# Newiz430/CellSegmentation

Measured on AMD Instinct MI355X. Metric: tiles/sec fwd+bwd (ResNet-50 MIL, 299x299), higher is better.
Workload: dtype bf16; 1 GPU; ResNet-50 tile classifier (train_tile.py --scratch semantics: fwd + CE + full bwd + Adam), bag=64 tiles of 299x299x3 per GPU, freeze_bn=True; tiles_per_gpu=64, parallelism=dp1

## Files before the change

### cellsegmentation_amd/_lib.py

```python
import ctypes
import os
from ctypes import POINTER, Structure, c_char_p, c_double, c_float, c_int, c_int32, c_int64, c_longlong, c_size_t, c_void_p

_HERE = os.path.dirname(os.path.abspath(__file__))
FLAVOUR = os.environ.get("CELLSEG_LIB_FLAVOUR", "")
if FLAVOUR not in ("", "ab"):
    raise RuntimeError(f"CELLSEG_LIB_FLAVOUR={FLAVOUR!r}: expected unset or 'ab'")
LIB_PATH = os.path.join(_HERE, f"libcellseg_hip_{FLAVOUR}.so" if FLAVOUR else "libcellseg_hip.so")

CS_F32, CS_BF16 = 0, 1
CS_ACT_NONE, CS_ACT_RELU, CS_ACT_SILU, CS_ACT_SIGMOID = 0, 1, 2, 3
CS_BN_BWD_OWN_RELU, CS_BN_BWD_FROZEN = 0x100, 0x200


class CsConvGeom(Structure):
    _fields_ = [(n, c_int32) for n in ("N", "H", "W", "C", "K", "R", "S", "stride", "pad", "P", "Q", "groups")]


class CsStageDesc(Structure):
    _fields_ = ([(n, c_void_p) for n in ("w", "gamma", "beta", "mean", "var", "conv_bias", "w_khwc", "w_chwk", "scale", "shift", "rstd")]
                + [("eps", c_float)] + [(n, c_int32) for n in ("K", "Cin", "R", "S", "Cp", "Kp", "block0", "fwd_packed", "bwd_packed")])


class CellsegLibraryMissing(RuntimeError):
# ... 34 lines not shown
    "cs_conv2d_wgrad_batched_splits": (c_int, [POINTER(CsConvGeom), c_int, c_int]),
    "cs_conv2d_wgrad2_supported": (c_int, [POINTER(CsConvGeom), c_int]),
    "cs_conv2d_wgrad_batched": (c_int, [POINTER(CsConvGeom), c_int, _P, _P, _P, c_int, c_int, _P]),
    "cs_wgrad_finalize_batched": (c_int, [_P, _P, c_int, c_int, c_int, c_int, c_int, c_int, c_int, c_int, c_int, c_int, _P]),
    "cs_conv2d_dgrad_partial_rows": (c_int, [POINTER(CsConvGeom)]),
    "cs_fold_partial_rows": (c_int, [_P, c_int, c_int, _P, _P]),
    "cs_wgrad_finalize_grouped": (c_int, [_P, c_int, _P, _P, _P, _P, _P, c_int, c_int, c_int, c_int, _P, _P, _P, _P, _P]),
    "cs_colsum": (c_int, [_P, c_int, c_longlong, c_int, _P, _P]),
    "cs_colsum_partial_rows": (c_int, [c_longlong]),
    "cs_colsum_partial": (c_int, [_P, c_int, c_longlong, c_int, _P, _P]),
    "cs_positive_bits": (c_int, [_P, c_int, c_longlong, c_int, _P, _P]),
    "cs_adam_chunk_elems": (c_int, []),
    "cs_adam_max_tensors": (c_int, []),
    "cs_adam_step": (c_int, [_P, _P, c_int, c_int, _P, c_int, c_double, c_double, c_double, c_double, c_double, c_double, _P]),
    "cs_adam_step_dev": (c_int, [_P, _P, c_int, c_int, _P, c_int, _P, _P, _P, c_double, c_double, c_double, c_double, c_double, _P]),
    "cs_sgd_step": (c_int, [_P, _P, c_int, c_int, _P, c_int, c_double, c_double, c_double, c_double, c_int, c_int, _P]),
    "cs_sgd_step_dev": (c_int, [_P, _P, c_int, c_int, _P, c_int, _P, c_double, c_double, c_int, c_int, _P]),
    "cs_sample_sum_workspace": (c_size_t, [c_int, c_int, c_int]),
    "cs_sample_sum": (c_int, [_P, _P, c_int, c_float, _P, _P, c_int, c_int, c_int, _P]),
    "cs_maxpool3x3s2_fwd": (c_int, [_P, c_int, _P, _P, c_int, c_int, c_int, c_int, c_int, c_int, _P]),
    "cs_maxpool3x3s2_bwd": (c_int, [_P, _P, _P, c_int, _P, c_int, c_int, c_int, c_int, c_int, c_int, _P]),
    "cs_gap_avgmax_fwd": (c_int, [_P, c_int, _P, _P, c_int, c_int, c_int, c_int, _P]),
    "cs_gap_avgmax_bwd": (c_int, [_P, _P, _P, c_int, _P, c_int, c_int, c_int, c_int, c_int, _P]),
    "cs_linear_fwd": (c_int, [_P, _P, _P, _P, _P, c_int, c_int, c_int, c_int, _P]),
    "cs_linear_bwd_workspace": (c_size_t, [c_int, c_int, c_int]),
    "cs_linear_bwd": (c_int, [_P, _P, _P, _P, c_int, _P, _P, _P, c_int, c_int, c_int, c_int, _P, _P]),
    "cs_loss_words": (c_int, []),
    "cs_softmax_ce": (c_int, [_P, _P, c_float, _P, _P, c_int, c_int, _P]),
    "cs_softmax_prob1": (c_int, [_P, _P, c_int, c_int, _P]),
    "cs_softmax_argmax": (c_int, [_P, _P, c_int, c_int, _P]),
    "cs_mse": (c_int, [_P, _P, c_int, c_int, _P, _P, c_int, _P]),
    "cs_bn_accum_words": (c_size_t, [c_int]),
    "cs_bn_accum_read": (c_int, [_P, c_int, _P, _P]),
    "cs_bn_stats": (c_int, [_P, c_int, c_longlong, c_int, _P, _P, _P]),
    "cs_bn_partial_workspace": (c_size_t, [c_longlong, c_int]),
    "cs_bn_finalize": (c_int, [_P, c_longlong, c_float, c_float, _P, _P, _P, _P, c_int, _P]),
    "cs_bn_apply": (c_int, [_P, c_int, _P, _P, _P, _P, _P, c_int, _P, c_longlong, c_int, _P]),
    "cs_bn_apply_stats": (c_int, [_P, c_int, _P, c_float, c_float, _P, _P, _P, _P, _P, c_int, _P, _P, _P, c_longlong, c_int, _P]),
    "cs_bn_bwd_reduce": (c_int, [_P, _P, c_int, _P, _P, _P, _P, c_int, c_longlong, c_int, _P, _P, _P]),
    "cs_bn_bwd_apply": (c_int, [_P, _P, c_int, _P, _P, _P, _P, c_int, _P, c_longlong, c_int, _P, _P, _P, _P]),
    "cs_dwconv_fwd": (c_int, [POINTER(CsConvGeom), c_int, _P, _P, _P, _P, c_int, _P, _P]),
    "cs_dwconv_fwd_stats_workspace": (c_size_t, [POINTER(CsConvGeom)]),
    "cs_dwconv_fwd_stats": (c_int, [POINTER(CsConvGeom), c_int, _P, _P, _P, _P, POINTER(c_int), _P]),
    "cs_bn_partial_fold": (c_int, [_P, c_int, c_int, _P, _P]),
    "cs_dwconv_dgrad": (c_int, [POINTER(CsConvGeom), c_int, _P, _P, _P, _P]),
    "cs_dwconv_wgrad": (c_int, [POINTER(CsConvGeom), c_int, _P, _P, _P, _P, _P]),
# ... 143 lines not shown
```

### cellsegmentation_amd/csrc/pool.hip

```cpp
#include "cs_common.h"

namespace {

template <typename T>
__global__ __launch_bounds__(256) void maxpool_fwd_kernel(const T* __restrict__ x, T* __restrict__ y,
                                                          uint8_t* __restrict__ amax, int N, int H, int W, int C, int P,
                                                          int Q) {
    const int CG = C / 8;
    const long long total = (long long)N * P * Q * CG;
    for (long long idx = (long long)blockIdx.x * blockDim.x + threadIdx.x; idx < total;
         idx += (long long)gridDim.x * blockDim.x) {
        const int cg = (int)(idx % CG);
        long long t = idx / CG;
        const int q = (int)(t % Q); t /= Q;
        const int p = (int)(t % P);
        const long long n = t / P;
        float best[8];
        int bi[8];
#pragma unroll
        for (int e = 0; e < 8; ++e) { best[e] = -INFINITY; bi[e] = 0; }
        bool first = true;
#pragma unroll
        for (int kh = 0; kh < 3; ++kh) {
            const int iy = p * 2 - 1 + kh;
// ... 2 lines not shown
            for (int kw = 0; kw < 3; ++kw) {
                const int ix = q * 2 - 1 + kw;
                if (ix < 0 || ix >= W) continue;
                float v[8];
                load8<T>(x + ((n * H + iy) * (long long)W + ix) * C + cg * 8, v);
#pragma unroll
                for (int e = 0; e < 8; ++e) {
                    if (first || v[e] > best[e] || v[e] != v[e]) { best[e] = v[e]; bi[e] = kh * 3 + kw; }
                }
                first = false;
            }
        }
        const long long o = ((n * P + p) * (long long)Q + q) * C + cg * 8;
        store8<T>(y + o, best);
        if (amax) {
            uint2 pk;
            pk.x = (uint32_t)bi[0] | ((uint32_t)bi[1] << 8) | ((uint32_t)bi[2] << 16) | ((uint32_t)bi[3] << 24);
            pk.y = (uint32_t)bi[4] | ((uint32_t)bi[5] << 8) | ((uint32_t)bi[6] << 16) | ((uint32_t)bi[7] << 24);
            *reinterpret_cast<uint2*>(amax + o) = pk;
        }
    }
}

template <typename T>
__global__ __launch_bounds__(256) void maxpool_bwd_block_kernel(const T* __restrict__ dy, const uint8_t* __restrict__ amax,
                                                                const T* __restrict__ y, T* __restrict__ dx, int N, int H, int W,
                                                                int C, int P, int Q) {
    const int CG = C / 8;
    const int Ha = (H + 1) / 2, Wb = (W + 1) / 2;
    const long long total = (long long)N * Ha * Wb * CG;
    for (long long idx = (long long)blockIdx.x * blockDim.x + threadIdx.x; idx < total;
         idx += (long long)gridDim.x * blockDim.x) {
        const int cg = (int)(idx % CG);
        long long t = idx / CG;
        const int b = (int)(t % Wb); t /= Wb;
        const int a = (int)(t % Ha);
        const long long n = t / Ha;
        float acc[2][2][8];
#pragma unroll
        for (int i = 0; i < 2; ++i)
#pragma unroll
            for (int j = 0; j < 2; ++j)
#pragma unroll
                for (int e = 0; e < 8; ++e) acc[i][j][e] = 0.f;
#pragma unroll
        for (int wp = 0; wp < 2; ++wp) {
            const int p = a + wp;
            if (p >= P) continue;
#pragma unroll
            for (int wq = 0; wq < 2; ++wq) {
                const int q = b + wq;
// ... 6 lines not shown
                    float yy[8];
                    load8<T>(y + o, yy);
#pragma unroll
                    for (int e = 0; e < 8; ++e) g[e] = yy[e] > 0.f ? g[e] : 0.f;
                }
#pragma unroll
                for (int i = 0; i < 2; ++i) {
                    const int kh = i + 1 - 2 * wp;
                    if (kh < 0 || kh > 2) continue;
#pragma unroll
                    for (int j = 0; j < 2; ++j) {
                        const int kw = j + 1 - 2 * wq;
                        if (kw < 0 || kw > 2) continue;
                        const uint32_t want = (uint32_t)(kh * 3 + kw);
#pragma unroll
                        for (int e = 0; e < 8; ++e) {
                            const uint32_t am = ((e < 4 ? pk.x : pk.y) >> (8 * (e & 3))) & 0xffu;
                            if (am == want) acc[i][j][e] += g[e];
                        }
                    }
                }
            }
        }
#pragma unroll
        for (int i = 0; i < 2; ++i) {
            const int iy = 2 * a + i;
            if (iy >= H) continue;
#pragma unroll
            for (int j = 0; j < 2; ++j) {
                const int ix = 2 * b + j;
                if (ix < W) store8<T>(dx + ((n * H + iy) * (long long)W + ix) * C + cg * 8, acc[i][j]);
            }
        }
    }
}

template <typename T>
__global__ __launch_bounds__(256) void gap_fwd_kernel(const T* __restrict__ x, float* __restrict__ feat,
                                                      int32_t* __restrict__ amax, int HW, int C, int with_max) {
    const int CG = C / 8;
    const int n = blockIdx.y;
    const int cg = blockIdx.x * 64 + (threadIdx.x & 63);
    const int part = threadIdx.x >> 6;
    __shared__ float s_sum[4][64][8];
    __shared__ float s_max[4][64][8];
    __shared__ int s_idx[4][64][8];
    float sum[8], mx[8];
    int mi[8];
#pragma unroll
    for (int e = 0; e < 8; ++e) { sum[e] = 0.f; mx[e] = -INFINITY; mi[e] = 0x7fffffff; }
    if (cg < CG) {
        const T* base = x + (long long)n * HW * C + cg * 8;
        int p = part;
        for (; p + 12 < HW; p += 16) {
            float v[4][8];
#pragma unroll
            for (int u = 0; u < 4; ++u) load8<T>(base + (long long)(p + 4 * u) * C, v[u]);
// ... 19 lines not shown
    for (int e = 0; e < 8; ++e) {
        s_sum[part][threadIdx.x & 63][e] = sum[e];
        s_max[part][threadIdx.x & 63][e] = mx[e];
        s_idx[part][threadIdx.x & 63][e] = mi[e];
    }
    __syncthreads();
    if (part == 0 && cg < CG) {
        const int l = threadIdx.x & 63;
#pragma unroll
        for (int e = 0; e < 8; ++e) {
            float s = 0.f, m = -INFINITY;
            int bi = 0x7fffffff;
            for (int q = 0; q < 4; ++q) {
                s += s_sum[q][l][e];
                const float mq = s_max[q][l][e];
                const int iq = s_idx[q][l][e];
                if (iq == 0x7fffffff) continue;
                const bool nq = mq != mq, nm = m != m;
                if (bi == 0x7fffffff || (nq ? (!nm || iq > bi) : (!nm && (mq > m || (mq == m && iq < bi))))) { m = mq; bi = iq; }
            }
            feat[(long long)n * C + cg * 8 + e] = s / (float)HW + (with_max ? m : 0.f);
            if (amax) amax[(long long)n * C + cg * 8 + e] = bi;
        }
    }
}

template <typename T>
__global__ __launch_bounds__(256) void gap_bwd_kernel(const float* __restrict__ dfeat, const int32_t* __restrict__ amax,
                                                      const T* __restrict__ x, T* __restrict__ dx, int N, int HW, int C,
                                                      int relu_mask, int with_max) {
    const int CG = C / 8;
    const long long total = (long long)N * HW * CG;
    const float inv = 1.f / (float)HW;
    for (long long idx = (long long)blockIdx.x * blockDim.x + threadIdx.x; idx < total;
         idx += (long long)gridDim.x * blockDim.x) {
        const int cg = (int)(idx % CG);
        const long long t = idx / CG;
        const int p = (int)(t % HW);
        const long long n = t / HW;
        float v[8], g8[8];
        load8p(dfeat + n * C + cg * 8, 0.f, g8);
        int am[8];
        if (with_max) {
            const int4 a0 = *reinterpret_cast<const int4*>(amax + n * C + cg * 8);
            const int4 a1 = *reinterpret_cast<const int4*>(amax + n * C + cg * 8 + 4);
            am[0] = a0.x; am[1] = a0.y; am[2] = a0.z; am[3] = a0.w; am[4] = a1.x; am[5] = a1.y; am[6] = a1.z; am[7] = a1.w;
        }
#pragma unroll
        for (int e = 0; e < 8; ++e) v[e] = g8[e] * inv + ((with_max && am[e] == p) ? g8[e] : 0.f);
        const long long o = (n * HW + p) * C + cg * 8;
        if (relu_mask) {
            float xx[8];
            load8<T>(x + o, xx);
#pragma unroll
            for (int e = 0; e < 8; ++e) v[e] = xx[e] > 0.f ? v[e] : 0.f;
        }
        store8<T>(dx + o, v);
    }
}

inline int grid_for(long long total) {
    long long b = (total + 255) / 256;
    if (b > 16384) b = 16384;
    if (b < 1) b = 1;
    return (int)b;
}

}

extern "C" int cs_maxpool3x3s2_fwd(const void* x, int dtype, void* y, uint8_t* argmax, int N, int H, int W, int C, int P,
                                   int Q, void* stream) {
    CS_CHECK_ARG(x && y, "maxpool_fwd: NULL tensor");
    CS_CHECK_ARG(C > 0 && C % 8 == 0, "maxpool_fwd: C must be a multiple of 8");
    CS_CHECK_ARG(P == (H + 2 - 3) / 2 + 1 && Q == (W + 2 - 3) / 2 + 1, "maxpool_fwd: P/Q do not match H/W");
    hipStream_t st = reinterpret_cast<hipStream_t>(stream);
    const long long total = (long long)N * P * Q * (C / 8);
    return cs_launch_typed(dtype, "maxpool_fwd", [&](auto tc) {
        using T = typename decltype(tc)::type;
        hipLaunchKernelGGL(maxpool_fwd_kernel<T>, dim3(grid_for(total)), dim3(256), 0, st, (const T*)x, (T*)y, argmax, N, H, W, C, P, Q);
    });
}

extern "C" int cs_maxpool3x3s2_bwd(const void* dy, const uint8_t* argmax, const void* y_mask, int dtype, void* dx, int N,
                                   int H, int W, int C, int P, int Q, void* stream) {
    CS_CHECK_ARG(dy && argmax && dx, "maxpool_bwd: NULL tensor");
    CS_CHECK_ARG(C > 0 && C % 8 == 0, "maxpool_bwd: C must be a multiple of 8");
    CS_CHECK_ARG(P == (H + 2 - 3) / 2 + 1 && Q == (W + 2 - 3) / 2 + 1, "maxpool_bwd: P/Q do not match H/W");
    hipStream_t st = reinterpret_cast<hipStream_t>(stream);
    const long long total = (long long)N * ((H + 1) / 2) * ((W + 1) / 2) * (C / 8);
    return cs_launch_typed(dtype, "maxpool_bwd", [&](auto tc) {
        using T = typename decltype(tc)::type;
        hipLaunchKernelGGL(maxpool_bwd_block_kernel<T>, dim3(grid_for(total)), dim3(256), 0, st, (const T*)dy, argmax, (const T*)y_mask, (T*)dx, N, H, W, C, P, Q);
    });
}

extern "C" int cs_gap_avgmax_fwd(const void* x, int dtype, float* feat, int32_t* argmax, int N, int HW, int C, int with_max,
                                 void* stream) {
    CS_CHECK_ARG(x && feat, "gap_fwd: NULL tensor");
    CS_CHECK_ARG(N > 0 && HW > 0 && C > 0 && C % 8 == 0, "gap_fwd: bad extents");
    hipStream_t st = reinterpret_cast<hipStream_t>(stream);
    dim3 grid((C / 8 + 63) / 64, N);
    return cs_launch_typed(dtype, "gap_fwd", [&](auto tc) {
        using T = typename decltype(tc)::type;
        hipLaunchKernelGGL(gap_fwd_kernel<T>, grid, dim3(256), 0, st, (const T*)x, feat, argmax, HW, C, with_max);
    });
}

extern "C" int cs_gap_avgmax_bwd(const float* dfeat, const int32_t* argmax, const void* x, int dtype, void* dx, int N, int HW,
                                 int C, int relu_mask, int with_max, void* stream) {
    CS_CHECK_ARG(dfeat && dx && (argmax || !with_max), "gap_bwd: NULL tensor");
    CS_CHECK_ARG(!relu_mask || x, "gap_bwd: relu_mask needs x");
    CS_CHECK_ARG(N > 0 && HW > 0 && C > 0 && C % 8 == 0, "gap_bwd: bad extents");
    hipStream_t st = reinterpret_cast<hipStream_t>(stream);
    const long long total = (long long)N * HW * (C / 8);
    return cs_launch_typed(dtype, "gap_bwd", [&](auto tc) {
        using T = typename decltype(tc)::type;
        hipLaunchKernelGGL(gap_bwd_kernel<T>, dim3(grid_for(total)), dim3(256), 0, st, dfeat, argmax, (const T*)x, (T*)dx, N, HW, C, relu_mask, with_max);
    });
}
```

### cellsegmentation_amd/engine.py

```python
from collections import namedtuple
from types import SimpleNamespace

import torch

from . import _capture
from . import kernels as K

ACT_NONE, ACT_RELU, ACT_SILU = K.CS_ACT_NONE, K.CS_ACT_RELU, K.CS_ACT_SILU

PACKED = True
PACKED_TRAIN_BN = True
FUSE_STEM_POOL = True


class ConvUnit:
    kind = "conv"

    def __init__(self, name, conv, bn, act, src, dst, res=None):
        self.name, self.conv, self.bn, self.act = name, conv, bn, act
        self.src, self.dst, self.res = src, dst, res
        self.grouped = conv.groups != 1
        if self.grouped:
            cg = conv.in_channels // conv.groups
            if conv.in_channels != conv.out_channels or conv.in_channels % 64 != 0 or 64 % cg != 0 or conv.bias is not None:
                raise NotImplementedError(f"{name}: grouped convolution needs C == K, C % 64 == 0, (C/groups) | 64, no bias "
                                          "(the ResNeXt 32x4d / 32x8d 3x3 layers)")
        self._cache = None

    def params(self):
        out = [("weight", self.conv.weight)]
        if self.conv.bias is not None:
            out.append(("bias", self.conv.bias))
        if self.bn is not None:
            out += [("gamma", self.bn.weight), ("beta", self.bn.bias)]
        return out
# ... 194 lines not shown
class PoolUnit:
    kind = "pool"

    def __init__(self, src, dst):
        self.src, self.dst = src, dst

    def params(self):
        return []

    def inputs(self):
        return [self.src]

    def fwd(self, f, ui):
        if f.aux[ui] is not None:
            return
        x = f.t[self.src]
        f.t[self.dst], am = K.maxpool_fwd(x, want_argmax=f.save)
        f.aux[ui] = SimpleNamespace(argmax=am, in_hw=tuple(x.shape[1:3]))

    def bwd(self, b, ui, g):
        if b.requires.get(self.src, False):
            b.sole_consumer(self.src, "pool")
            a = b.aux[ui]
            b.grads[self.src] = K.maxpool_bwd(g, a.argmax, None, a.in_hw)


class UpsampleUnit:
    kind = "up"

    def __init__(self, src, dst, size_like=None, size_fn=None):
        self.src, self.dst, self.size_like, self.size_fn = src, dst, size_like, size_fn

    def params(self):
        return []

    def inputs(self):
        return [self.src]

    def fwd(self, f, ui):
        x = f.t[self.src]
        size = tuple(f.t[self.size_like].shape[1:3]) if self.size_like is not None else tuple(self.size_fn(f.in_hw))
        f.t[self.dst] = K.bilinear_fwd(x, size)
        f.aux[ui] = SimpleNamespace(in_hw=tuple(x.shape[1:3]))

    def bwd(self, b, ui, g):
        if b.requires.get(self.src, False):
            b.sole_consumer(self.src, "upsample")
# ... 364 lines not shown
        if self.need(ui, "beta"):
            self.emit(ui, "beta", dbeta if n is None else dbeta[:n])

    def grad_buffer(self, param):
        v = self.sink.view_for(param) if self.sink is not None else None
        return v if v is not None else torch.empty_like(param)

    def take(self, n):
        v = self.arena.take(n)
        return v if v is not None else torch.zeros((n,), dtype=torch.float32, device=self.dev)

    def contribute(self, slot, g, masked):
        self.left[slot] -= 1
        if slot in self.grads:
            raise NotImplementedError("engine: unfused gradient accumulation is not expected for these networks")
        if self.left[slot] == 0 and slot in self.plan.relu_slots and not masked:
            raise NotImplementedError("engine: last contribution to a post-ReLU slot must come from a masking kernel")
        self.grads[slot] = g

    def sole_consumer(self, slot, what):
        self.left[slot] -= 1
        if slot in self.grads:
            raise NotImplementedError(f"engine: {what} input with several consumers")

    def bn_bwd(self, ui, u, g, a, n=None):
        bn, want = u.bn, self.need(ui, "gamma") or self.need(ui, "beta")
        dz, dgamma, dbeta = K.bn_bwd(g, a.z, a.mean, a.rstd, bn.weight.detach(), want_param_grads=want, beta=bn.bias.detach(),
                                     act=ACT_SILU if u.act == ACT_SILU else ACT_NONE)
        self.emit_bn(ui, dgamma, dbeta, n)
        return dz

    def colsums(self, u, a, g, dz, partial):
        cached = self.gsum_cache.pop(u.dst, None) if not a.train else None
        if partial:
            gsum = cached if cached is not None else K.colsum_partial(dz)
        else:
            gsum = K.colsum_vector(cached) if cached is not None else K.colsum(dz)
        if not a.train and u.res is not None and self.grads.get(u.res) is g:
            self.gsum_cache[u.res] = gsum
        return gsum

    def defer_wgrad(self, ui, u, a, x, g, dz):
        gsum = None
        if not a.train:
            gsum = self.colsums(u, a, g, dz, partial=True)
        elif self.need(ui, "bias"):
# ... 73 lines not shown
        if st.bwd_packed and geom.stride != 1:
            if final or pending is not None:
                raise RuntimeError(f"{u.name}: compact strided data gradient out of order (it must be the first contribution)")
            return K.conv_dgrad_packed(geom, dz, st.w_chwk)
        if st.bwd_packed:
            if mask is not None and a.train:
                mbits, mask = K.positive_bits(mask), None
            if mask is not None:
                raise RuntimeError(f"{u.name}: packed data-gradient operand staged but the ReLU mask is not a bit tensor")
            if not final:
                return K.conv_dgrad_packed(geom, dz, st.w_chwk, add=pending, mask_bits=mbits)
            dx, self.gsum_cache[u.src] = K.conv_dgrad_packed(geom, dz, st.w_chwk, add=pending, mask_bits=mbits, want_colsum=True)
            return dx
        if isinstance(pending, K.CompactGrad):
            raise RuntimeError(f"{u.name}: a compact gradient reached a data gradient that cannot add it")
        if not final:
            return K.conv_dgrad(geom, dz, st.w_chwk, add=pending, mask=mask, grouped=u.grouped, mask_bits=mbits)
        cs = self.take(geom.C) if (geom.stride != 1 or u.grouped) else None
        dx, self.gsum_cache[u.src] = K.conv_dgrad(geom, dz, st.w_chwk, add=pending, mask=mask, colsum=cs, grouped=u.grouped,
                                                  defer_colsum=True, mask_bits=mbits)
        return dx


def backward(plan, state, grad_feeds, param_needs, requires, use_tr_read=True):
    b = _Backward(plan, state, grad_feeds, param_needs, requires, use_tr_read)
    for ui in reversed(range(len(plan.units))):
        u = plan.units[ui]
        g = b.grads.pop(u.dst, None)
        if g is not None:
            u.bwd(b, ui, g)
    for items in list(b.deferred.values()):
        b.flush(items)
    return {s: b.grads.get(s) for s in plan.inputs}, b.pgrads


class _PlanFunction(torch.autograd.Function):
    @staticmethod
    def forward(ctx, plan, cfg, n_inputs, *tensors):
        inputs, params = tensors[:n_inputs], tensors[n_inputs:]
        feeds = {s: x for s, x in zip(plan.inputs, inputs)}
        input_needs = {s: ctx.needs_input_grad[3 + i] for i, s in enumerate(plan.inputs)}
        param_needs = [ctx.needs_input_grad[3 + n_inputs + i] for i in range(len(params))]
        save = any(param_needs) or any(input_needs.values())
        requires, _ = compute_requires(plan, param_needs, input_needs)
        state = forward(plan, feeds, cfg.dtype, cfg.bn_train, save, requires, cfg.image_hw, getattr(cfg, "input_nchw", None))
        ctx.plan, ctx.cfg, ctx.n_inputs = plan, cfg, n_inputs
        ctx.param_needs, ctx.requires = param_needs, requires
        ctx.state = state if save else None
        outs = tuple(state.t[s] for s in plan.outputs)
        return outs

    @staticmethod
    def backward(ctx, *gouts):
        plan = ctx.plan
        grad_feeds = {}
        for s, g in zip(plan.outputs, gouts):
            if g is not None:
                grad_feeds[s] = g.contiguous()
        in_grads, pgrads = backward(plan, ctx.state, grad_feeds, ctx.param_needs, ctx.requires, ctx.cfg.use_tr_read)
        ctx.state = None
        return (None, None, None) + tuple(in_grads[s] for s in plan.inputs) + tuple(pgrads)


def run_plan(plan, inputs, dtype, bn_train, use_tr_read=True, image_hw=None, input_nchw=None):
    cfg = SimpleNamespace(dtype=dtype, bn_train=bn_train, use_tr_read=use_tr_read, image_hw=image_hw, input_nchw=None)
    if input_nchw is not None:
        if len(plan.inputs) != 1 or input_nchw.requires_grad or input_nchw.dtype != torch.float32 or input_nchw.dim() != 4 or input_nchw.shape[1] != 3:
            raise ValueError("run_plan: input_nchw is a single fp32 [N,3,H,W] image without gradient")
        cfg.input_nchw = input_nchw.contiguous()
        N, _, H, W = input_nchw.shape
        inputs = [torch.empty((N, H, W, K.pad_channels(3)), dtype=dtype, device=input_nchw.device)]
    return _PlanFunction.apply(plan, cfg, len(inputs), *inputs, *plan.param_tensors())
```

### cellsegmentation_amd/functional.py

```python
import torch

from . import kernels as K


class _ToNHWC(torch.autograd.Function):
    @staticmethod
    def forward(ctx, x, dtype, Cp):
        ctx.C = x.shape[1]
        return K.to_nhwc(x.contiguous(), dtype, Cp)

    @staticmethod
    def backward(ctx, g):
        return K.to_nchw(g.contiguous(), ctx.C), None, None


def to_nhwc(x, dtype, Cp=None):
    return _ToNHWC.apply(x, dtype, Cp or K.pad_channels(x.shape[1]))


class _ToNCHW(torch.autograd.Function):
    @staticmethod
    def forward(ctx, y, C):
        ctx.dtype, ctx.Cp = y.dtype, y.shape[-1]
        return K.to_nchw(y, C)

    @staticmethod
    def backward(ctx, g):
        return K.to_nhwc(g.contiguous(), ctx.dtype, ctx.Cp), None


def to_nchw(y, C):
    return _ToNCHW.apply(y, C)


class _GapAvgMax(torch.autograd.Function):

    @staticmethod
    def forward(ctx, x, C, relu_input):
        feat, am = K.gap_fwd(x)
        ctx.save_for_backward(x, am)
        ctx.C, ctx.relu_input = C, relu_input
        return feat[:, :C] if C != feat.shape[1] else feat

    @staticmethod
    def backward(ctx, g):
        x, am = ctx.saved_tensors
        Cp = x.shape[-1]
        if g.shape[1] != Cp:
            gp = torch.zeros((g.shape[0], Cp), dtype=g.dtype, device=g.device)
            gp[:, : g.shape[1]] = g
            g = gp
        return K.gap_bwd(g.contiguous(), am, x, ctx.relu_input), None, None


def gap_avgmax(x_nhwc, C, relu_input=True):
    return _GapAvgMax.apply(x_nhwc, C, relu_input)


class _Linear(torch.autograd.Function):
    @staticmethod
    def forward(ctx, x, w, b, act):
        x = x.contiguous()
        y = K.linear_fwd(x, w.detach().contiguous(), b.detach().contiguous() if b is not None else None, act)
        ctx.save_for_backward(x, w, y)
        ctx.act, ctx.has_b = act, b is not None
        return y

    @staticmethod
    def backward(ctx, g):
        x, w, y = ctx.saved_tensors
        need_dx, need_dw = ctx.needs_input_grad[0], ctx.needs_input_grad[1]
        need_db = ctx.has_b and ctx.needs_input_grad[2]
        dx, dw, db = K.linear_bwd(x, w.detach().contiguous(), g.contiguous(), y, ctx.act, need_dx, need_dw or need_db, need_db)
        return dx, (dw if need_dw else None), (db if need_db else None), None

# ... 135 lines not shown
```

### cellsegmentation_amd/kernels.py

```python
import ctypes

import torch

from . import _lib
from ._lib import (CS_ACT_NONE, CS_ACT_RELU, CS_ACT_SIGMOID, CS_ACT_SILU, CS_BF16, CS_BN_BWD_FROZEN, CS_BN_BWD_OWN_RELU, CS_F32,
                   CsConvGeom)


def _code(dtype):
    if dtype == torch.float32:
        return CS_F32
    if dtype == torch.bfloat16:
        return CS_BF16
    raise TypeError(f"unsupported activation dtype {dtype}; use torch.float32 or torch.bfloat16")


def _f32(*tensors):
    for t in tensors:
        if t.dtype != torch.float32:
            raise TypeError(f"this kernel reads torch.float32 only, got {t.dtype}; cast on the way in (functional.py does)")


def chunk(dtype):
    return 4 if dtype == torch.float32 else 8
# ... 744 lines not shown
def se_scale_bwd_dx(dy, s, davg):
    N, H, W, C = dy.shape
    dx = torch.empty_like(dy)
    _lib.check(_lib.load().cs_se_scale_bwd_dx(_p(dy), _code(dy.dtype), _p(s), _p(davg), _p(dx), N, H * W, C, _stream()), "se_scale_bwd_dx")
    return dx


def rowscale_add(a, row_scale, b):
    N = a.shape[0]
    y = torch.empty_like(a)
    _lib.check(_lib.load().cs_rowscale_add(_p(a), _code(a.dtype), _p(row_scale), _p(b), _p(y), N, a.numel() // N, _stream()), "rowscale_add")
    return y


def maxpool_fwd(x, want_argmax=True):
    N, H, W, C = x.shape
    P, Q = (H - 1) // 2 + 1, (W - 1) // 2 + 1
    y = torch.empty((N, P, Q, C), dtype=x.dtype, device=x.device)
    am = torch.empty((N, P, Q, C), dtype=torch.uint8, device=x.device) if want_argmax else None
    _lib.check(_lib.load().cs_maxpool3x3s2_fwd(_p(x), _code(x.dtype), _p(y), _p(am), N, H, W, C, P, Q, _stream()), "maxpool_fwd")
    return y, am


def maxpool_bwd(dy, argmax, y_mask, in_hw):
    N, P, Q, C = dy.shape
    H, W = in_hw
    dx = torch.empty((N, H, W, C), dtype=dy.dtype, device=dy.device)
    _lib.check(_lib.load().cs_maxpool3x3s2_bwd(_p(dy), _p(argmax), _p(y_mask), _code(dy.dtype), _p(dx), N, H, W, C, P, Q,
                                               _stream()), "maxpool_bwd")
    return dx


def gap_fwd(x, with_max=True):
    N, H, W, C = x.shape
    if not with_max:
        return sample_sum(x, None, 1.0 / (H * W)), None
    feat = torch.empty((N, C), dtype=torch.float32, device=x.device)
    am = torch.empty((N, C), dtype=torch.int32, device=x.device) if with_max else None
    _lib.check(_lib.load().cs_gap_avgmax_fwd(_p(x), _code(x.dtype), _p(feat), _p(am), N, H * W, C, 1 if with_max else 0, _stream()),
               "gap_fwd")
    return feat, am


def gap_bwd(dfeat, argmax, x, relu_mask, with_max=True):
    N, H, W, C = x.shape
    dx = torch.empty_like(x)
    _lib.check(_lib.load().cs_gap_avgmax_bwd(_p(dfeat), _p(argmax), _p(x), _code(x.dtype), _p(dx), N, H * W, C,
                                             1 if relu_mask else 0, 1 if with_max else 0, _stream()), "gap_bwd")
    return dx


_LOSS_WORDS = 16
def linear_fwd(x, w, b, act=CS_ACT_NONE, want_preact=False):
    M, K = x.shape
    N = w.shape[0]
    y = torch.empty((M, N), dtype=torch.float32, device=x.device)
    pre = torch.empty_like(y) if want_preact else None
    _lib.check(_lib.load().cs_linear_fwd(_p(x), _p(w), _p(b), _p(y), _p(pre), M, N, K, act, _stream()), "linear_fwd")
    return (y, pre) if want_preact else y


def linear_bwd(x, w, dy, y=None, act=CS_ACT_NONE, need_dx=True, need_dw=True, need_db=True):
    M, K = x.shape
    N = w.shape[0]
    dx = torch.empty((M, K), dtype=torch.float32, device=x.device) if need_dx else None
    dw = torch.empty((N, K), dtype=torch.float32, device=x.device) if (need_dw or need_db) else None
    db = torch.empty((N,), dtype=torch.float32, device=x.device) if need_db else None
    lib = _lib.load()
    nws = lib.cs_linear_bwd_workspace(M, N, K) if dw is not None else 0
    ws = torch.empty((nws // 4,), dtype=torch.float32, device=x.device) if nws else None
    _lib.check(lib.cs_linear_bwd(_p(x), _p(w), _p(dy), _p(y), act, _p(dx), _p(dw), _p(db), M, N, K, 0, _p(ws), _stream()),
               "linear_bwd")
# ... 1062 lines not shown
```

### include/cellseg_hip.h

```cpp
#ifndef CELLSEG_HIP_H_
#define CELLSEG_HIP_H_

#include <stdint.h>
#include <stddef.h>

#ifdef __cplusplus
extern "C" {
#endif

enum { CS_F32 = 0, CS_BF16 = 1 };
enum { CS_OK = 0, CS_ERR_INVALID_ARG = -1, CS_ERR_LAUNCH = -2, CS_ERR_UNSUPPORTED = -3 };
enum { CS_ACT_NONE = 0, CS_ACT_RELU = 1, CS_ACT_SILU = 2, CS_ACT_SIGMOID = 3 };

int cs_abi_version(void);
const char* cs_last_error(void);
const char* cs_last_conv_variant(void);

typedef struct CsConvGeom {
    int32_t N, H, W, C;
    int32_t K;
    int32_t R, S;
    int32_t stride, pad;
    int32_t P, Q;
    int32_t groups;
// ... 83 lines not shown
int cs_adam_step_dev(const CsAdamTensor* tensors_dev, const void* const* grads_host, int t0, int n_tensors, const int* chunks_dev,
                     int n_chunks, float* const* steps_dev, float* coef_dev, const double* lr_dev, double lr, double beta1, double beta2,
                     double eps, double weight_decay, void* stream);
typedef struct CsSgdTensor { float* p; float* buf; long long n; } CsSgdTensor;
int cs_sgd_step(const CsSgdTensor* tensors_dev, const void* const* grads_host, int t0, int n_tensors, const int* chunks_dev, int n_chunks,
                double lr, double momentum, double dampening, double weight_decay, int nesterov, int first, void* stream);
int cs_sgd_step_dev(const CsSgdTensor* tensors_dev, const void* const* grads_host, int t0, int n_tensors, const int* chunks_dev, int n_chunks,
                    const double* hyper_dev, double dampening, double weight_decay, int nesterov, int first, void* stream);

size_t cs_sample_sum_workspace(int N, int HW, int C);
int cs_sample_sum(const void* a, const void* b, int dtype, float scale, float* out, float* workspace, int N, int HW, int C,
                  void* stream);
int cs_positive_bits(const void* x, int dtype, long long n_pixels, int C, uint8_t* bits, void* stream);
int cs_colsum_partial(const void* g, int dtype, long long M, int C, float* partial, void* stream);

int cs_maxpool3x3s2_fwd(const void* x, int dtype, void* y, uint8_t* argmax, int N, int H, int W, int C, int P, int Q,
                        void* stream);
int cs_maxpool3x3s2_bwd(const void* dy, const uint8_t* argmax, const void* y_mask, int dtype, void* dx, int N, int H,
                        int W, int C, int P, int Q, void* stream);
int cs_gap_avgmax_fwd(const void* x, int dtype, float* feat, int32_t* argmax, int N, int HW, int C, int with_max,
                      void* stream);
int cs_gap_avgmax_bwd(const float* dfeat, const int32_t* argmax, const void* x, int dtype, void* dx, int N, int HW,
                      int C, int relu_mask, int with_max, void* stream);

int cs_bilinear_ac_fwd(const void* x, int dtype, void* y, int N, int H, int W, int C, int P, int Q, void* stream);
int cs_bilinear_ac_bwd(const void* dy, const void* mask, int dtype, void* dx, int N, int H, int W, int C, int P, int Q,
                       void* stream);
int cs_concat_channels(const void* a, const void* b, int dtype, void* out, long long M, int Ca, int Cb, void* stream);
int cs_split_channels(const void* whole, int dtype, void* a, void* b, long long M, int Ca, int Cb, void* stream);

int cs_dwconv_fwd(const CsConvGeom* g, int dtype, const void* x, const float* w_hwc, const float* scale, const float* shift,
                  int act, void* y, void* stream);
size_t cs_dwconv_fwd_stats_workspace(const CsConvGeom* g);
int cs_dwconv_fwd_stats(const CsConvGeom* g, int dtype, const void* x, const float* w_hwc, void* y, double* partial,
                        int* partial_rows, void* stream);
int cs_bn_partial_fold(const double* partial, int rows, int C, double* stats, void* stream);
int cs_dwconv_dgrad(const CsConvGeom* g, int dtype, const void* dy, const float* w_hwc, void* dx, void* stream);
size_t cs_dwconv_wgrad_workspace(const CsConvGeom* g);
int cs_dwconv_wgrad(const CsConvGeom* g, int dtype, const void* x, const void* dy, float* dw_hwc, float* workspace, void* stream);
int cs_dwconv_wgrad_oihw(const CsConvGeom* g, int dtype, const void* x, const void* dy, float* dw_oihw, float* workspace, void* stream);
typedef struct { const float* src; float* dst; long long C; long long RS; long long first; } CsDwStageDesc;
int cs_dw_weights_hwc_multi(const CsDwStageDesc* desc_dev, int n, long long total, void* stream);
int cs_se_scale(const void* x, int dtype, const float* s, void* y, int N, int HW, int C, void* stream);
int cs_se_scale_bwd_dx(const void* dy, int dtype, const float* s, const float* davg, void* dx, int N, int HW, int C, void* stream);
int cs_rowscale_add(const void* a, int dtype, const float* row_scale, const void* b, void* y, int N, long long per_row,
                    void* stream);
// ... 230 lines not shown
```

Measured before the change: 9627 tiles/s.

## Fuse per-channel gradient column sums into maxpool and GAP backward producers

Maxpool backward and global-avg/max-pool backward kernels can now also emit per-block partial column sums of the gradient they write. The engine passes these partials on to the downstream frozen-BN beta/gamma reduction, so that reduction no longer has to reread the full gradient tensor. The GAP case crosses the autograd boundary through a weakref-keyed offer cache. This adds shared-memory reductions and a partial buffer to those kernels, plus cache-validation logic that could silently fall back or go stale.

```diff
diff --git a/cellsegmentation_amd/_lib.py b/cellsegmentation_amd/_lib.py
--- a/cellsegmentation_amd/_lib.py
+++ b/cellsegmentation_amd/_lib.py
@@ -80,6 +80,10 @@
     "cs_maxpool3x3s2_bwd": (c_int, [_P, _P, _P, c_int, _P, c_int, c_int, c_int, c_int, c_int, c_int, _P]),
     "cs_gap_avgmax_fwd": (c_int, [_P, c_int, _P, _P, c_int, c_int, c_int, c_int, _P]),
     "cs_gap_avgmax_bwd": (c_int, [_P, _P, _P, c_int, _P, c_int, c_int, c_int, c_int, c_int, _P]),
+    "cs_maxpool3x3s2_bwd_colsum_rows": (c_int, [c_int, c_int, c_int, c_int]),
+    "cs_maxpool3x3s2_bwd_colsum": (c_int, [_P, _P, _P, c_int, _P, c_int, c_int, c_int, c_int, c_int, c_int, _P, _P]),
+    "cs_gap_avgmax_bwd_colsum_rows": (c_int, [c_int, c_int, c_int]),
+    "cs_gap_avgmax_bwd_colsum": (c_int, [_P, _P, _P, c_int, _P, c_int, c_int, c_int, c_int, c_int, _P, _P]),
     "cs_linear_fwd": (c_int, [_P, _P, _P, _P, _P, c_int, c_int, c_int, c_int, _P]),
     "cs_linear_bwd_workspace": (c_size_t, [c_int, c_int, c_int]),
     "cs_linear_bwd": (c_int, [_P, _P, _P, _P, c_int, _P, _P, _P, c_int, c_int, c_int, c_int, _P, _P]),
diff --git a/cellsegmentation_amd/csrc/pool.hip b/cellsegmentation_amd/csrc/pool.hip
--- a/cellsegmentation_amd/csrc/pool.hip
+++ b/cellsegmentation_amd/csrc/pool.hip
@@ -48,11 +48,64 @@
     }
 }
 
-template <typename T>
-__global__ __launch_bounds__(256) void maxpool_bwd_block_kernel(const T* __restrict__ dy, const uint8_t* __restrict__ amax,
+template <typename T> __device__ __forceinline__ void store8_stored(T* p, const float (&v)[8], float (&r)[8]);
+template <> __device__ __forceinline__ void store8_stored<float>(float* p, const float (&v)[8], float (&r)[8]) {
+    store8<float>(p, v);
+#pragma unroll
+    for (int e = 0; e < 8; ++e) r[e] = v[e];
+}
+template <> __device__ __forceinline__ void store8_stored<bf16_t>(bf16_t* p, const float (&v)[8], float (&r)[8]) {
+    uint4 o;
+    o.x = pack_bf16x2(v[0], v[1]);
+    o.y = pack_bf16x2(v[2], v[3]);
+    o.z = pack_bf16x2(v[4], v[5]);
+    o.w = pack_bf16x2(v[6], v[7]);
+    *reinterpret_cast<uint4*>(p) = o;
+    r[0] = __uint_as_float(o.x << 16); r[1] = __uint_as_float(o.x & 0xffff0000u);
+    r[2] = __uint_as_float(o.y << 16); r[3] = __uint_as_float(o.y & 0xffff0000u);
+    r[4] = __uint_as_float(o.z << 16); r[5] = __uint_as_float(o.z & 0xffff0000u);
+    r[6] = __uint_as_float(o.w << 16); r[7] = __uint_as_float(o.w & 0xffff0000u);
+}
+
+__device__ __forceinline__ void store_partial_row(float (*fold)[256], float* __restrict__ stage , int width,
+                                                  float* __restrict__ partial, long long row, int C, int c0) {
+    __syncthreads();
+    const int ncols = width * 8;
+    if (ncols >= 256) {
+        const int rpar = 256 / width;
+        for (int col = threadIdx.x; col < ncols; col += 256) {
+            const int cgl = col % width, e = col / width;
+            float t = 0.f;
+            for (int r = 0; r < rpar; ++r) t += fold[e][r * width + cgl];
+            partial[row * 2 * C + c0 + cgl * 8 + e] = t;
+        }
+    } else {
+        const int col = threadIdx.x % ncols, seg = threadIdx.x / ncols, nseg = 256 / ncols;
+        const int cgl = col % width, e = col / width;
+        float t = 0.f;
+#pragma unroll
+        for (int r = 0; r < 8; ++r) t += fold[e][(seg * 8 + r) * width + cgl];
+        stage[threadIdx.x] = t;
+        __syncthreads();
+        if (seg == 0) {
+            t = 0.f;
+            for (int s = 0; s < nseg; ++s) t += stage[s * ncols + col];
+            partial[row * 2 * C + c0 + cgl * 8 + e] = t;
+        }
+    }
+}
+
+template <typename T, bool COLSUM>
+__global__ __launch_bounds__(256, COLSUM ? 6 : 1) void maxpool_bwd_block_kernel(const T* __restrict__ dy, const uint8_t* __restrict__ amax,
                                                                 const T* __restrict__ y, T* __restrict__ dx, int N, int H, int W,
-                                                                int C, int P, int Q) {
+                                                                int C, int P, int Q, float* __restrict__ partial) {
     const int CG = C / 8;
+    __shared__ float s_cs[COLSUM ? 8 : 1][256];
+    __shared__ float s_stage[COLSUM ? 256 : 1];
+    if constexpr (COLSUM) {
+#pragma unroll
+        for (int e = 0; e < 8; ++e) s_cs[e][threadIdx.x] = 0.f;
+    }
     const int Ha = (H + 1) / 2, Wb = (W + 1) / 2;
     const long long total = (long long)N * Ha * Wb * CG;
     for (long long idx = (long long)blockIdx.x * blockDim.x + threadIdx.x; idx < total;
@@ -105,6 +158,9 @@
                 }
             }
         }
+        float cs[8];
+#pragma unroll
+        for (int e = 0; e < 8; ++e) cs[e] = 0.f;
 #pragma unroll
         for (int i = 0; i < 2; ++i) {
             const int iy = 2 * a + i;
@@ -112,10 +168,24 @@
 #pragma unroll
             for (int j = 0; j < 2; ++j) {
                 const int ix = 2 * b + j;
-                if (ix < W) store8<T>(dx + ((n * H + iy) * (long long)W + ix) * C + cg * 8, acc[i][j]);
+                if (ix >= W) continue;
+                T* o = dx + ((n * H + iy) * (long long)W + ix) * C + cg * 8;
+                if constexpr (COLSUM) {
+                    float r[8];
+                    store8_stored<T>(o, acc[i][j], r);
+#pragma unroll
+                    for (int e = 0; e < 8; ++e) cs[e] += r[e];
+                } else {
+                    store8<T>(o, acc[i][j]);
+                }
             }
         }
-    }
+        if constexpr (COLSUM) {
+#pragma unroll
+            for (int e = 0; e < 8; ++e) s_cs[e][threadIdx.x] += cs[e];
+        }
+    }
+    if constexpr (COLSUM) store_partial_row(s_cs, s_stage, CG, partial, blockIdx.x, C, 0);
 }
 
 template <typename T>
@@ -181,6 +251,21 @@
             feat[(long long)n * C + cg * 8 + e] = s / (float)HW + (with_max ? m : 0.f);
             if (amax) amax[(long long)n * C + cg * 8 + e] = bi;
         }
+    }
+}
+
+__device__ __forceinline__ void gap_bwd_value(const float (&g8)[8], const int (&am)[8], int p, float inv, int with_max, float (&v)[8]) {
+#pragma unroll
+    for (int e = 0; e < 8; ++e) v[e] = g8[e] * inv + ((with_max && am[e] == p) ? g8[e] : 0.f);
+}
+
+__device__ __forceinline__ void gap_bwd_sample(const float* __restrict__ dfeat, const int32_t* __restrict__ amax, long long o,
+                                               int with_max, float (&g8)[8], int (&am)[8]) {
+    load8p(dfeat + o, 0.f, g8);
+    if (with_max) {
+        const int4 a0 = *reinterpret_cast<const int4*>(amax + o);
+        const int4 a1 = *reinterpret_cast<const int4*>(amax + o + 4);
+        am[0] = a0.x; am[1] = a0.y; am[2] = a0.z; am[3] = a0.w; am[4] = a1.x; am[5] = a1.y; am[6] = a1.z; am[7] = a1.w;
     }
 }
 
@@ -198,15 +283,9 @@
         const int p = (int)(t % HW);
         const long long n = t / HW;
         float v[8], g8[8];
-        load8p(dfeat + n * C + cg * 8, 0.f, g8);
         int am[8];
-        if (with_max) {
-            const int4 a0 = *reinterpret_cast<const int4*>(amax + n * C + cg * 8);
-            const int4 a1 = *reinterpret_cast<const int4*>(amax + n * C + cg * 8 + 4);
-            am[0] = a0.x; am[1] = a0.y; am[2] = a0.z; am[3] = a0.w; am[4] = a1.x; am[5] = a1.y; am[6] = a1.z; am[7] = a1.w;
-        }
-#pragma unroll
-        for (int e = 0; e < 8; ++e) v[e] = g8[e] * inv + ((with_max && am[e] == p) ? g8[e] : 0.f);
+        gap_bwd_sample(dfeat, amax, n * C + cg * 8, with_max, g8, am);
+        gap_bwd_value(g8, am, p, inv, with_max, v);
         const long long o = (n * HW + p) * C + cg * 8;
         if (relu_mask) {
             float xx[8];
@@ -216,6 +295,49 @@
         }
         store8<T>(dx + o, v);
     }
+}
+
+template <typename T>
+__global__ __launch_bounds__(256) void gap_bwd_colsum_kernel(const float* __restrict__ dfeat, const int32_t* __restrict__ amax,
+                                                             const T* __restrict__ x, T* __restrict__ dx, float* __restrict__ partial,
+                                                             long long M, int HW, int C, int width, int run, int relu_mask,
+                                                             int with_max) {
+    const int lanes = 256 / width;
+    const int cg = blockIdx.x * width + (int)(threadIdx.x % width);
+    const int pl = threadIdx.x / width;
+    const long long m0 = (long long)blockIdx.y * run;
+    const long long m1 = m0 + run < M ? m0 + run : M;
+    const float inv = 1.f / (float)HW;
+    float cs[8], g8[8];
+    int am[8];
+#pragma unroll
+    for (int e = 0; e < 8; ++e) { cs[e] = 0.f; g8[e] = 0.f; am[e] = -1; }
+    long long n_cur = -1;
+    for (long long m = m0 + pl; m < m1; m += lanes) {
+        const long long n = m / HW;
+        const int p = (int)(m - n * HW);
+        if (n != n_cur) {
+            gap_bwd_sample(dfeat, amax, n * C + cg * 8, with_max, g8, am);
+            n_cur = n;
+        }
+        float v[8], r[8];
+        gap_bwd_value(g8, am, p, inv, with_max, v);
+        const long long o = m * C + cg * 8;
+        if (relu_mask) {
+            float xx[8];
+            load8<T>(x + o, xx);
+#pragma unroll
+            for (int e = 0; e < 8; ++e) v[e] = xx[e] > 0.f ? v[e] : 0.f;
+        }
+        store8_stored<T>(dx + o, v, r);
+#pragma unroll
+        for (int e = 0; e < 8; ++e) cs[e] += r[e];
+    }
+    __shared__ float s_cs[8][256];
+    __shared__ float s_stage[256];
+#pragma unroll
+    for (int e = 0; e < 8; ++e) s_cs[e][threadIdx.x] = cs[e];
+    store_partial_row(s_cs, s_stage, width, partial, blockIdx.y, C, blockIdx.x * width * 8);
 }
 
 inline int grid_for(long long total) {
@@ -249,7 +371,7 @@
     const long long total = (long long)N * ((H + 1) / 2) * ((W + 1) / 2) * (C / 8);
     return cs_launch_typed(dtype, "maxpool_bwd", [&](auto tc) {
         using T = typename decltype(tc)::type;
-        hipLaunchKernelGGL(maxpool_bwd_block_kernel<T>, dim3(grid_for(total)), dim3(256), 0, st, (const T*)dy, argmax, (const T*)y_mask, (T*)dx, N, H, W, C, P, Q);
+        hipLaunchKernelGGL((maxpool_bwd_block_kernel<T, false>), dim3(grid_for(total)), dim3(256), 0, st, (const T*)dy, argmax, (const T*)y_mask, (T*)dx, N, H, W, C, P, Q, (float*)nullptr);
     });
 }
 
@@ -277,3 +399,63 @@
         hipLaunchKernelGGL(gap_bwd_kernel<T>, dim3(grid_for(total)), dim3(256), 0, st, dfeat, argmax, (const T*)x, (T*)dx, N, HW, C, relu_mask, with_max);
     });
 }
+
+namespace {
+
+constexpr int kPoolColsumMaxRows = 4096;
+constexpr int kGapColsumWidth = 16;
+constexpr int kGapColsumMinRun = 40;
+constexpr int kGapColsumRows = 128;
+
+inline bool colsum_channels_served(int C) { return C >= 8 && C <= 2048 && (C & (C - 1)) == 0; }
+
+inline int gap_colsum_run(long long M) {
+    long long run = (M + kGapColsumRows - 1) / kGapColsumRows;
+    return (int)(run < kGapColsumMinRun ? kGapColsumMinRun : run);
+}
+
+}
+
+extern "C" int cs_maxpool3x3s2_bwd_colsum_rows(int N, int H, int W, int C) {
+    if (N <= 0 || H <= 0 || W <= 0 || !colsum_channels_served(C)) return 0;
+    const long long total = (long long)N * ((H + 1) / 2) * ((W + 1) / 2) * (C / 8);
+    const long long b = (total + 255) / 256;
+    return (int)(b > kPoolColsumMaxRows ? kPoolColsumMaxRows : b);
+}
+
+extern "C" int cs_maxpool3x3s2_bwd_colsum(const void* dy, const uint8_t* argmax, const void* y_mask, int dtype, void* dx, int N,
+                                          int H, int W, int C, int P, int Q, float* partial, void* stream) {
+    CS_CHECK_ARG(dy && argmax && dx && partial, "maxpool_bwd_colsum: NULL tensor");
+    CS_CHECK_ARG(P == (H + 2 - 3) / 2 + 1 && Q == (W + 2 - 3) / 2 + 1, "maxpool_bwd_colsum: P/Q do not match H/W");
+    const int rows = cs_maxpool3x3s2_bwd_colsum_rows(N, H, W, C);
+    CS_CHECK_ARG(rows > 0, "maxpool_bwd_colsum: shape not served (C must be a power of two in 8..2048)");
+    hipStream_t st = reinterpret_cast<hipStream_t>(stream);
+    return cs_launch_typed(dtype, "maxpool_bwd_colsum", [&](auto tc) {
+        using T = typename decltype(tc)::type;
+        hipLaunchKernelGGL((maxpool_bwd_block_kernel<T, true>), dim3(rows), dim3(256), 0, st, (const T*)dy, argmax, (const T*)y_mask, (T*)dx, N, H, W, C, P, Q, partial);
+    });
+}
+
+extern "C" int cs_gap_avgmax_bwd_colsum_rows(int N, int HW, int C) {
+    if (N <= 0 || HW <= 0 || !colsum_channels_served(C)) return 0;
+    const long long M = (long long)N * HW;
+    const int run = gap_colsum_run(M);
+    return (int)((M + run - 1) / run);
+}
+
+extern "C" int cs_gap_avgmax_bwd_colsum(const float* dfeat, const int32_t* argmax, const void* x, int dtype, void* dx, int N, int HW,
+                                        int C, int relu_mask, int with_max, float* partial, void* stream) {
+    CS_CHECK_ARG(dfeat && dx && partial && (argmax || !with_max), "gap_bwd_colsum: NULL tensor");
+    CS_CHECK_ARG(!relu_mask || x, "gap_bwd_colsum: relu_mask needs x");
+    const int rows = cs_gap_avgmax_bwd_colsum_rows(N, HW, C);
+    CS_CHECK_ARG(rows > 0, "gap_bwd_colsum: shape not served (C must be a power of two in 8..2048)");
+    hipStream_t st = reinterpret_cast<hipStream_t>(stream);
+    const long long M = (long long)N * HW;
+    const int CG = C / 8;
+    const int width = CG < kGapColsumWidth ? CG : kGapColsumWidth;
+    dim3 grid(CG / width, rows);
+    return cs_launch_typed(dtype, "gap_bwd_colsum", [&](auto tc) {
+        using T = typename decltype(tc)::type;
+        hipLaunchKernelGGL(gap_bwd_colsum_kernel<T>, grid, dim3(256), 0, st, dfeat, argmax, (const T*)x, (T*)dx, partial, M, HW, C, width, gap_colsum_run(M), relu_mask, with_max);
+    });
+}
diff --git a/cellsegmentation_amd/engine.py b/cellsegmentation_amd/engine.py
--- a/cellsegmentation_amd/engine.py
+++ b/cellsegmentation_amd/engine.py
@@ -1,3 +1,4 @@
+import weakref
 from collections import namedtuple
 from types import SimpleNamespace
 
@@ -11,6 +12,7 @@
 PACKED = True
 PACKED_TRAIN_BN = True
 FUSE_STEM_POOL = True
+PRODUCER_COLSUMS = True
 
 
 class ConvUnit:
@@ -251,7 +253,10 @@
         if b.requires.get(self.src, False):
             b.sole_consumer(self.src, "pool")
             a = b.aux[ui]
-            b.grads[self.src] = K.maxpool_bwd(g, a.argmax, None, a.in_hw)
+            if PRODUCER_COLSUMS and b.wants_colsums(self.src):
+                b.grads[self.src], b.gsum_cache[self.src] = K.maxpool_bwd(g, a.argmax, None, a.in_hw, want_colsum=True)
+            else:
+                b.grads[self.src] = K.maxpool_bwd(g, a.argmax, None, a.in_hw)
 
 
 class UpsampleUnit:
@@ -662,6 +667,14 @@
         self.left[slot] -= 1
         if slot in self.grads:
             raise NotImplementedError(f"engine: {what} input with several consumers")
+
+    def wants_colsums(self, slot):
+        for ui, u in enumerate(self.plan.units):
+            if u.dst == slot:
+                a = self.aux[ui]
+                return (u.kind == "conv" and u.bn is not None and a is not None and not a.train
+                        and bool(self.need(ui, "gamma") or self.need(ui, "beta")))
+        return False
 
     def bn_bwd(self, ui, u, g, a, n=None):
         bn, want = u.bn, self.need(ui, "gamma") or self.need(ui, "beta")
@@ -781,8 +794,32 @@
         return dx
 
 
-def backward(plan, state, grad_feeds, param_needs, requires, use_tr_read=True):
+_colsum_offers = {}
+
+
+def offer_colsum(grad, partial):
+    if PRODUCER_COLSUMS and partial is not None:
+        for k in [k for k, o in _colsum_offers.items() if o[0]() is None]:
+            del _colsum_offers[k]
+        _colsum_offers[(grad.data_ptr(), grad.numel())] = (weakref.ref(grad), grad._version, partial)
+
+
+def _take_colsum_offer(g):
+    offer = _colsum_offers.get((g.data_ptr(), g.numel()))
+    if offer is None:
+        return None
+    t = offer[0]()
+    if t is None or t.data_ptr() != g.data_ptr() or t.shape != g.shape or t.dtype != g.dtype or t._version != offer[1] \
+            or g._version != offer[1]:
+        return None
+    return offer[2]
+
+
+def backward(plan, state, grad_feeds, param_needs, requires, use_tr_read=True, gsum_seeds=None):
     b = _Backward(plan, state, grad_feeds, param_needs, requires, use_tr_read)
+    for s, ps in (gsum_seeds or {}).items():
+        if b.wants_colsums(s):
+            b.gsum_cache[s] = ps
     for ui in reversed(range(len(plan.units))):
         u = plan.units[ui]
         g = b.grads.pop(u.dst, None)
@@ -812,11 +849,17 @@
     @staticmethod
     def backward(ctx, *gouts):
         plan = ctx.plan
-        grad_feeds = {}
-        for s, g in zip(plan.outputs, gouts):
-            if g is not None:
-                grad_feeds[s] = g.contiguous()
-        in_grads, pgrads = backward(plan, ctx.state, grad_feeds, ctx.param_needs, ctx.requires, ctx.cfg.use_tr_read)
+        grad_feeds, seeds = {}, {}
+        try:
+            for s, g in zip(plan.outputs, gouts):
+                if g is not None:
+                    grad_feeds[s] = g.contiguous()
+                    ps = _take_colsum_offer(grad_feeds[s]) if _colsum_offers else None
+                    if ps is not None:
+                        seeds[s] = ps
+        finally:
+            _colsum_offers.clear()
+        in_grads, pgrads = backward(plan, ctx.state, grad_feeds, ctx.param_needs, ctx.requires, ctx.cfg.use_tr_read, seeds)
         ctx.state = None
         return (None, None, None) + tuple(in_grads[s] for s in plan.inputs) + tuple(pgrads)
 
diff --git a/cellsegmentation_amd/functional.py b/cellsegmentation_amd/functional.py
--- a/cellsegmentation_amd/functional.py
+++ b/cellsegmentation_amd/functional.py
@@ -1,5 +1,6 @@
 import torch
 
+from . import engine as E
 from . import kernels as K
 
 
@@ -31,6 +32,14 @@
 
 def to_nchw(y, C):
     return _ToNCHW.apply(y, C)
+
+
+def _gap_bwd_offering(g, am, x, relu_input):
+    if not (E.PRODUCER_COLSUMS and K.gap_bwd_leaves_colsums(x)):
+        return K.gap_bwd(g, am, x, relu_input)
+    dx, partial = K.gap_bwd(g, am, x, relu_input, want_colsum=True)
+    E.offer_colsum(dx, partial)
+    return dx
 
 
 class _GapAvgMax(torch.autograd.Function):
@@ -50,7 +59,7 @@
             gp = torch.zeros((g.shape[0], Cp), dtype=g.dtype, device=g.device)
             gp[:, : g.shape[1]] = g
             g = gp
-        return K.gap_bwd(g.contiguous(), am, x, ctx.relu_input), None, None
+        return _gap_bwd_offering(g.contiguous(), am, x, ctx.relu_input), None, None
 
 
 def gap_avgmax(x_nhwc, C, relu_input=True):
diff --git a/cellsegmentation_amd/kernels.py b/cellsegmentation_amd/kernels.py
--- a/cellsegmentation_amd/kernels.py
+++ b/cellsegmentation_amd/kernels.py
@@ -790,13 +790,20 @@
     return y, am
 
 
-def maxpool_bwd(dy, argmax, y_mask, in_hw):
+def maxpool_bwd(dy, argmax, y_mask, in_hw, want_colsum=False):
     N, P, Q, C = dy.shape
     H, W = in_hw
     dx = torch.empty((N, H, W, C), dtype=dy.dtype, device=dy.device)
-    _lib.check(_lib.load().cs_maxpool3x3s2_bwd(_p(dy), _p(argmax), _p(y_mask), _code(dy.dtype), _p(dx), N, H, W, C, P, Q,
-                                               _stream()), "maxpool_bwd")
-    return dx
+    lib = _lib.load()
+    rows = lib.cs_maxpool3x3s2_bwd_colsum_rows(N, H, W, C) if want_colsum else 0
+    if rows > 0:
+        buf = torch.empty((rows, 2 * C), dtype=torch.float32, device=dy.device)
+        _lib.check(lib.cs_maxpool3x3s2_bwd_colsum(_p(dy), _p(argmax), _p(y_mask), _code(dy.dtype), _p(dx), N, H, W, C, P, Q, _p(buf),
+                                                  _stream()), "maxpool_bwd_colsum")
+        return dx, PartialColsum(buf, rows, C)
+    _lib.check(lib.cs_maxpool3x3s2_bwd(_p(dy), _p(argmax), _p(y_mask), _code(dy.dtype), _p(dx), N, H, W, C, P, Q, _stream()),
+               "maxpool_bwd")
+    return (dx, colsum_partial(dx)) if want_colsum else dx
 
 
 def gap_fwd(x, with_max=True):
@@ -810,12 +817,24 @@
     return feat, am
 
 
-def gap_bwd(dfeat, argmax, x, relu_mask, with_max=True):
+def gap_bwd_leaves_colsums(x):
+    N, H, W, C = x.shape
+    return _lib.load().cs_gap_avgmax_bwd_colsum_rows(N, H * W, C) > 0
+
+
+def gap_bwd(dfeat, argmax, x, relu_mask, with_max=True, want_colsum=False):
     N, H, W, C = x.shape
     dx = torch.empty_like(x)
-    _lib.check(_lib.load().cs_gap_avgmax_bwd(_p(dfeat), _p(argmax), _p(x), _code(x.dtype), _p(dx), N, H * W, C,
-                                             1 if relu_mask else 0, 1 if with_max else 0, _stream()), "gap_bwd")
-    return dx
+    lib = _lib.load()
+    rows = lib.cs_gap_avgmax_bwd_colsum_rows(N, H * W, C) if want_colsum else 0
+    if rows > 0:
+        buf = torch.empty((rows, 2 * C), dtype=torch.float32, device=x.device)
+        _lib.check(lib.cs_gap_avgmax_bwd_colsum(_p(dfeat), _p(argmax), _p(x), _code(x.dtype), _p(dx), N, H * W, C,
+                                                1 if relu_mask else 0, 1 if with_max else 0, _p(buf), _stream()), "gap_bwd_colsum")
+        return dx, PartialColsum(buf, rows, C)
+    _lib.check(lib.cs_gap_avgmax_bwd(_p(dfeat), _p(argmax), _p(x), _code(x.dtype), _p(dx), N, H * W, C,
+                                     1 if relu_mask else 0, 1 if with_max else 0, _stream()), "gap_bwd")
+    return (dx, colsum_partial(dx)) if want_colsum else dx
 
 
 _LOSS_WORDS = 16
diff --git a/include/cellseg_hip.h b/include/cellseg_hip.h
--- a/include/cellseg_hip.h
+++ b/include/cellseg_hip.h
@@ -129,6 +129,12 @@
                       void* stream);
 int cs_gap_avgmax_bwd(const float* dfeat, const int32_t* argmax, const void* x, int dtype, void* dx, int N, int HW,
                       int C, int relu_mask, int with_max, void* stream);
+int cs_maxpool3x3s2_bwd_colsum_rows(int N, int H, int W, int C);
+int cs_maxpool3x3s2_bwd_colsum(const void* dy, const uint8_t* argmax, const void* y_mask, int dtype, void* dx, int N, int H,
+                               int W, int C, int P, int Q, float* partial, void* stream);
+int cs_gap_avgmax_bwd_colsum_rows(int N, int HW, int C);
+int cs_gap_avgmax_bwd_colsum(const float* dfeat, const int32_t* argmax, const void* x, int dtype, void* dx, int N, int HW,
+                             int C, int relu_mask, int with_max, float* partial, void* stream);
 
 int cs_bilinear_ac_fwd(const void* x, int dtype, void* y, int N, int H, int W, int C, int P, int Q, void* stream);
 int cs_bilinear_ac_bwd(const void* dy, const void* mask, int dtype, void* dx, int N, int H, int W, int C, int P, int Q,
```

New measurement: 9660 tiles/s (median of 6 runs). No clear change (+0.3%).
